# pain7576/ddpg-trucktrailer

Measured on AMD Instinct MI355X. Metric: env-steps/s, higher is better.
Workload: dtype f64

## Files before the change

ddpg-trucktrailer_amd/csrc/ttnet_pack.h:

```cpp
#pragma once
#include "ttnet_common.h"

namespace ttnet {

using f32x16 = __attribute__((ext_vector_type(16))) float;
using f16x8 = __attribute__((ext_vector_type(8))) _Float16;
using h2 = __attribute__((ext_vector_type(2))) _Float16;

constexpr int ROWS = 128, WROWS = 32;
constexpr int T1 = 13, H1P = 32 * T1;
constexpr int T2 = 10, H2P = 32 * T2;
constexpr int STEPS = H1 / 16;
constexpr int S1 = 2;
constexpr int PIECES = 2 * T2;
constexpr int CHUNK_U4 = PIECES * 64;
constexpr int CHUNK_BYTES = CHUNK_U4 * 16;
constexpr int RING = 7;
constexpr int AHEAD = RING - 2;
constexpr int RING_BYTES = RING * CHUNK_BYTES;
constexpr int W1_PIECES = S1 * T1 * 2;
constexpr int W1_BYTES = W1_PIECES * 1024;
constexpr int W1_OFF = 2 * CHUNK_BYTES;
static_assert(W1_OFF + W1_BYTES <= AHEAD * CHUNK_BYTES, "packed fc1 must fit in the ring slots that are filled after layer 1");
constexpr int VEC_FLOATS = 2 * H1P + 6 * H2P;
constexpr int VEC_PIECES = 12;
constexpr int VEC_BYTES = VEC_PIECES * 1024;
constexpr int LDS_BYTES = RING_BYTES + VEC_BYTES;
constexpr int WS_W2 = 0, WS_W1 = STEPS * CHUNK_BYTES, WS_VEC = WS_W1 + W1_BYTES, WS_BYTES = WS_VEC + VEC_BYTES;

constexpr float SX = 16.f, SW = 64.f;
constexpr float UNSCALE = 1.f / (SX * SW);

__device__ __forceinline__ void split2(const float x0, const float x1, uint32_t &ph, uint32_t &pm) {
    h2 h;
    h[0] = (_Float16)x0; h[1] = (_Float16)x1;
    ph = __builtin_bit_cast(uint32_t, h);
    float r0, r1;
    asm("v_fma_mix_f32 %0, %1, -1.0, %2 op_sel_hi:[1,0,0]" : "=v"(r0) : "v"(ph), "v"(x0));
    asm("v_fma_mix_f32 %0, %1, -1.0, %2 op_sel:[1,0,0] op_sel_hi:[1,0,0]" : "=v"(r1) : "v"(ph), "v"(x1));
    h2 m;
    m[0] = (_Float16)r0; m[1] = (_Float16)r1;
    pm = __builtin_bit_cast(uint32_t, m);
}

using f32x2 = __attribute__((ext_vector_type(2))) float;
__device__ __forceinline__ f32x2 pk(const float a, const float b) { return f32x2{a, b}; }
__device__ __forceinline__ f32x2 pk_fma(const f32x2 a, const f32x2 b, const f32x2 c) { return __builtin_elementwise_fma(a, b, c); }

__device__ __forceinline__ f32x16 mfma_f16(const uint4 a, const uint4 b, const f32x16 c) {
    return __builtin_amdgcn_mfma_f32_32x32x16_f16(__builtin_bit_cast(f16x8, a), __builtin_bit_cast(f16x8, b), c, 0, 0, 0);
}

__device__ __forceinline__ void split_pack_body(const Weights &W, const bool critic, unsigned char *__restrict__ ws,
                                                unsigned char *__restrict__ ws_alt, long long *__restrict__ bump,
                                                const RingCursor &cur, const int idx) {
    if (ws_alt && cur.k_dev && (*cur.k_dev & 1)) ws = ws_alt;
    if (idx == 0) {
        if (bump) *bump += 1;
        write_cursor(cur);
    }
    constexpr int N2 = STEPS * T2 * 64, N1 = S1 * T1 * 64;
    if (idx < N2 + N1) {
        const bool l2 = idx < N2;
        const int q = l2 ? idx : idx - N2;
        const int lane = q & 63, su = q >> 6, nt = l2 ? T2 : T1, u = su % nt, s = su / nt;
        const int r = lane & 31, h = lane >> 5, row = 32 * u + r;
        float x[8];
        if (l2) {
#pragma unroll
            for (int g = 0; g < 2; ++g) {
                const float4 v = row < H2 ? *reinterpret_cast<const float4 *>(W.w2 + (size_t)row * H1 + 16 * s + 8 * g + 4 * h)
                                          : make_float4(0.f, 0.f, 0.f, 0.f);
                x[4 * g] = v.x; x[4 * g + 1] = v.y; x[4 * g + 2] = v.z; x[4 * g + 3] = v.w;
            }
        } else {
#pragma unroll
            for (int j = 0; j < 8; ++j) {
                const int k = 16 * s + 8 * h + j;
                x[j] = row < H1 ? (k < IN ? W.w1[row * IN + k] : (k == IN ? W.b1[row] : 0.f)) : 0.f;
            }
        }
        uint32_t ph[4], pm[4];
#pragma unroll
        for (int p = 0; p < 4; ++p) split2(x[2 * p] * SW, x[2 * p + 1] * SW, ph[p], pm[p]);
        uint4 *dst = reinterpret_cast<uint4 *>(ws + (l2 ? WS_W2 : WS_W1)) + ((size_t)su * 2) * 64 + lane;
        dst[0] = make_uint4(ph[0], ph[1], ph[2], ph[3]);
        dst[64] = make_uint4(pm[0], pm[1], pm[2], pm[3]);
        return;
    }
    const int i = idx - (N2 + N1);
    if (i >= VEC_BYTES / 4) return;
    float *vec = reinterpret_cast<float *>(ws + WS_VEC);
    float v = 0.f;
    if (i < 2 * H1P) {
        const int a = i / H1P, m = i % H1P;
        if (m < H1) v = (a == 0 ? W.g1[m] : W.be1[m]) * SX;
    } else if (i < VEC_FLOATS) {
        const int a = (i - 2 * H1P) / H2P, m = (i - 2 * H1P) % H2P;
        if (m < H2) {
            const float *src[6] = {W.b2, W.g2, W.be2, W.w3, W.wa, W.ba};
            if (a < 4 || critic) v = src[a][m];
        }
    } else if (i == VEC_FLOATS) {
        v = W.b3[0];
    }
    vec[i] = v;
}
constexpr int PACK_THREADS = (STEPS * T2 + S1 * T1) * 64 + VEC_BYTES / 4;
constexpr int PACK_BLOCKS = (PACK_THREADS + 255) / 256;


}
```

ddpg-trucktrailer_amd/csrc/ttnet_split.hip:

```cpp
#include "ttnet_common.h"
#include "ttnet_pack.h"
#include "ttstamps.h"

namespace ttnet {
namespace {

#ifdef TT_STAMPS
__device__ unsigned long long g_nstamps[16];
__device__ unsigned long long g_bstamps[4096 * 8];
#define NSTAMP(i) do { if (threadIdx.x == 0) { const unsigned long long w_ = wall_clock64();                                \
        if (blockIdx.x < 4096) { g_bstamps[blockIdx.x * 8 + (i)] = w_;                                                      \
            if ((i) == 0) g_bstamps[blockIdx.x * 8 + 7] = __builtin_amdgcn_s_getreg((20 << 0) | (0 << 6) | (3 << 11)); }     \
        if (blockIdx.x == 0) { g_nstamps[i] = w_; g_nstamps[8 + i] = clock64(); } } } while (0)
__device__ unsigned long long g_tile[512][4][2];
__device__ TTLog g_log_tile;
#define TSTAMP(round, e) do { if (threadIdx.x == 0 && blockIdx.x < 512 && (round) < 4) g_tile[blockIdx.x][round][e] = wall_clock64(); } while (0)
#else
#define NSTAMP(i) do { } while (0)
#define TSTAMP(round, e) do { } while (0)
#endif

__global__ __launch_bounds__(256) void k_split_pack(const Weights W, const bool critic, unsigned char *__restrict__ ws,
                                                    unsigned char *__restrict__ ws_alt, long long *__restrict__ bump,
                                                    const RingCursor cur) {
    split_pack_body(W, critic, ws, ws_alt, bump, cur, blockIdx.x * 256 + threadIdx.x);
    publish_image(cur, PACK_BLOCKS);
}

__global__ __launch_bounds__(256) void k_pack_and_sample(const Weights W, const bool critic, unsigned char *__restrict__ ws,
                                                         unsigned char *__restrict__ ws_alt, const RingSample R,
                                                         const RingCursor cur) {
    if ((int)blockIdx.x < PACK_BLOCKS) {
        split_pack_body(W, critic, ws, ws_alt, nullptr, cur, blockIdx.x * 256 + threadIdx.x);
        publish_image(cur, PACK_BLOCKS);
        return;
    }
    const int b = ((int)blockIdx.x - PACK_BLOCKS) * 4 + (threadIdx.x >> 6);
    if (b < R.batch * R.draws) ring_sample_row(R, b, threadIdx.x & 63);
}

using lds_b = const __attribute__((address_space(3))) unsigned char;
using v4u = __attribute__((ext_vector_type(4))) unsigned;
struct LdsBases {
    lds_b *b0, *b1, *b2;
};
__device__ __forceinline__ uint4 lds_frag(const LdsBases &L, const int off) {
    lds_b *p = (off >> 16) == 0 ? L.b0 : ((off >> 16) == 1 ? L.b1 : L.b2);
    const v4u t = *(const __attribute__((address_space(3))) v4u *)(p + (off & 0xFFFF));
    return make_uint4(t[0], t[1], t[2], t[3]);
}

template <bool CRITIC>
__global__ __launch_bounds__(256, 1) void k_mlp_split(const int n, const int tile0, const int tile_end,
                                                      int *__restrict__ cursor_e, const long long *__restrict__ step_e,
                                                      const float *__restrict__ obs,
                                                      const unsigned char *__restrict__ ws,
                                                      const unsigned char *__restrict__ ws_alt,
                                                      const float *__restrict__ action, float *__restrict__ out,
                                                      const ActArgs act) {
    extern __shared__ __attribute__((aligned(16))) unsigned char lds_raw[];
    const float *p1_s = reinterpret_cast<const float *>(lds_raw + RING_BYTES);
    const int tid = threadIdx.x, lane = tid & 63;
    const int wave = __builtin_amdgcn_readfirstlane(tid >> 6);
    const int r = lane & 31, h = lane >> 5;
    using lds_f = const __attribute__((address_space(3))) float;
    using v4 = __attribute__((ext_vector_type(4))) float;
    auto lds4 = [](lds_f *q) -> float4 {
        const v4 t = *(const __attribute__((address_space(3))) v4 *)q;
        return make_float4(t[0], t[1], t[2], t[3]);
    };
    lds_f *pv1_0 = (lds_f *)(p1_s + 4 * h);
    LdsBases LB0;
    LB0.b0 = (lds_b *)lds_raw + lane * 16;
    LB0.b1 = LB0.b0 + 65536;
    LB0.b2 = LB0.b0 + 131072;
    const EpochPair epochs = await_image_early(cursor_e);
    const long long kstep = cursor_e ? *step_e : 0;
    const bool odd = act.cursor && (kstep & 1);
    const bool local = act.cursor && act.ring_slots > 0;
    const int slot_t = local ? (int)(kstep % act.ring_slots) : 0;
    const float *obs_base = local ? obs + (size_t)slot_t * act.ring_n * IN : obs;
    const unsigned lds_base0 = (unsigned)(uintptr_t)(__attribute__((address_space(3))) unsigned char *)lds_raw;
    auto dma_piece = [&](const unsigned char *base, const unsigned voff, const unsigned lds_wave, const unsigned dst_const)
                         __attribute__((always_inline)) {
        unsigned keep;
        asm volatile("s_mov_b32 %0, m0\n\ts_add_u32 m0, %3, %4\n\ts_nop 0\n\tglobal_load_lds_dwordx4 %1, %2\n\ts_mov_b32 m0, %0"
                     : "=&s"(keep) : "v"(voff), "s"(base), "s"(lds_wave), "s"(dst_const) : "memory", "scc");
    };
    const unsigned voff_w2 = lane * 16 + wave * 5120 + WS_W2;
    const unsigned voff_w1 = lane * 16 + wave * (W1_PIECES / 4) * 1024 + WS_W1;
    const unsigned voff_vec = lane * 16 + wave * (VEC_PIECES / 4) * 1024 + WS_VEC;
    const unsigned ldsw_w2_0 = lds_base0 + wave * 5120, ldsw_w1_0 = lds_base0 + W1_OFF + wave * (W1_PIECES / 4) * 1024;
    auto issue_fc1 = [&](const unsigned char *w, const unsigned ldsw_w1) __attribute__((always_inline)) {
#pragma unroll
        for (int i = 0; i < W1_PIECES / 4; ++i) dma_piece(w, voff_w1 + i * 1024, ldsw_w1, i * 1024);
    };
    auto issue_step_piece = [&](const unsigned char *w, const unsigned ldsw_w2, const int s, const int i) __attribute__((always_inline)) {
        dma_piece(w, voff_w2 + s * CHUNK_BYTES + i * 1024, ldsw_w2, (s % RING) * CHUNK_BYTES + i * 1024);
    };
    float xo[S1][8];
    float ou_pre = 0.f;
    unsigned dp_pre = 0u;
    const bool with_noise = !CRITIC && act.ou != nullptr;
    const uint8_t *dprev = act.done_prev;
    float *araw = act.act_raw;
    auto load_obs = [&](const int tile) __attribute__((always_inline)) {
        const int row = tile * ROWS + wave * WROWS + r;
        const int rowc = row < n ? row : n - 1;
        const float *orow = obs_base + (size_t)rowc * IN;
#pragma unroll
        for (int s = 0; s < S1; ++s)
#pragma unroll
            for (int j = 0; j < 8; ++j) {
                const int k = 16 * s + 8 * h + j;
                xo[s][j] = orow[k < IN ? k : IN - 1];
            }
        if (with_noise) {
            ou_pre = act.ou[rowc];
            dp_pre = dprev ? (unsigned)dprev[rowc] : 0u;
        }
    };

    NSTAMP(0);
    int tile = tile0 + (int)blockIdx.x;
    if (tile >= tile_end) return;
    if (local) {
        const int sl = act.ring_slots;
        const int slot_prev = slot_t == 0 ? sl - 1 : slot_t - 1;
        dprev = kstep > 0 ? act.done_prev + (size_t)slot_prev * act.ring_n : nullptr;
        araw = act.act_raw + (size_t)slot_t * act.ring_n;
    }
    if (!act.cursor || local) load_obs(tile);
    await_image(act.cursor, act.step_dev, epochs);
    const unsigned char *wsl = (odd && ws_alt) ? ws_alt : ws;
    if (act.cursor && !local) {
        obs_base = resolve_obs(act, obs);
        const int *c = cursor_of(act);
        dprev = c[3] ? act.done_prev + (size_t)c[2] * act.ring_n : nullptr;
        araw = act.act_raw + (size_t)c[0] * act.ring_n;
        load_obs(tile);
    }
    const unsigned long long noise_step = act.step + (act.step_dev ? (unsigned long long)*act.step_dev : 0ull);
    if (act.cursor && tile0 == 0 && blockIdx.x == 0 && tid == 0)
        __hip_atomic_store(act.cursor + CUR_PROGRESS, (int)(kstep + 1), __ATOMIC_RELAXED, __HIP_MEMORY_SCOPE_AGENT);
    if (act.cursor && tile0 == 0 && blockIdx.x == 0 && tid < 4) {
        const int sl = act.ring_slots;
        act.cursor[tid] = !local ? cursor_of(act)[tid]
                                 : (tid == 0 ? slot_t : tid == 1 ? (slot_t + 1 == sl ? 0 : slot_t + 1)
                                                      : tid == 2 ? (slot_t == 0 ? sl - 1 : slot_t - 1) : (kstep > 0 ? 1 : 0));
    }
    issue_fc1(wsl, ldsw_w1_0);
#pragma unroll
    for (int i = 0; i < VEC_PIECES / 4; ++i)
        dma_piece(wsl, voff_vec + i * 1024, lds_base0 + RING_BYTES + wave * (VEC_PIECES / 4) * 1024, i * 1024);
#pragma unroll
    for (int i = 0; i < 10; ++i) issue_step_piece(wsl, ldsw_w2_0, i / 5, i % 5);
    bool first = true;
#ifdef TT_STAMPS
    int round = 0;
    if (threadIdx.x == 0 && blockIdx.x < 512) for (int q = 0; q < 4; ++q) g_tile[blockIdx.x][q][0] = g_tile[blockIdx.x][q][1] = 0ull;
    if (threadIdx.x == 0 && blockIdx.x < 512) g_tile[blockIdx.x][0][0] = wall_clock64();
#endif

#pragma unroll 1
    for (;;) {
        const unsigned char *wsl_cur = wsl;
        unsigned ldsw_w2 = ldsw_w2_0, ldsw_w1 = ldsw_w1_0;
        LdsBases LB = LB0;
        lds_f *pv1 = pv1_0;
        asm volatile("" : "+s"(wsl_cur), "+s"(ldsw_w2), "+s"(ldsw_w1), "+v"(LB.b0), "+v"(LB.b1), "+v"(LB.b2), "+v"(pv1));
        lds_f *pv2 = pv1 + 2 * H1P;
        const int row = tile * ROWS + wave * WROWS + r;
#pragma unroll
        for (int s = 0; s < S1; ++s)
#pragma unroll
            for (int j = 0; j < 8; ++j) {
                const int k = 16 * s + 8 * h + j;
                xo[s][j] = k < IN ? (row < n ? xo[s][j] : 0.f) : (k == IN ? 1.f : 0.f);
            }
        float ou_next = 0.f;
        if (with_noise) ou_next = ou_advance(row < n ? row : n - 1, ou_pre, dp_pre != 0u, act, noise_step);
        uint4 xb[S1][2];
#pragma unroll
        for (int s = 0; s < S1; ++s) {
            uint32_t ph[4], pm[4];
#pragma unroll
            for (int p = 0; p < 4; ++p) split2(xo[s][2 * p] * SX, xo[s][2 * p + 1] * SX, ph[p], pm[p]);
            xb[s][0] = make_uint4(ph[0], ph[1], ph[2], ph[3]);
            xb[s][1] = make_uint4(pm[0], pm[1], pm[2], pm[3]);
        }
        if (first) asm volatile("s_waitcnt vmcnt(10)" ::: "memory");
        else asm volatile("s_waitcnt vmcnt(0)" ::: "memory");
        __builtin_amdgcn_s_barrier();
        if (first) NSTAMP(1);

        f32x16 acc1[T1];
#pragma unroll
        for (int t = 0; t < T1; ++t) {
#pragma unroll
            for (int v = 0; v < 16; ++v) acc1[t][v] = 0.f;
#pragma unroll
            for (int s = 0; s < S1; ++s) {
                const uint4 ah = lds_frag(LB, W1_OFF + ((s * T1 + t) * 2) * 1024), am = lds_frag(LB, W1_OFF + ((s * T1 + t) * 2 + 1) * 1024);
                acc1[t] = mfma_f16(am, xb[s][0], acc1[t]);
                acc1[t] = mfma_f16(ah, xb[s][1], acc1[t]);
                acc1[t] = mfma_f16(ah, xb[s][0], acc1[t]);
            }
        }
        if (first) NSTAMP(2);
        __builtin_amdgcn_s_barrier();
#pragma unroll
        for (int i = 10; i < 5 * (AHEAD + 1); ++i) issue_step_piece(wsl_cur, ldsw_w2, i / 5, i % 5);
        uint32_t hb[STEPS][4], mb[STEPS][4];
        f32x2 nmean, rstdp;
        {
            f32x2 sp = pk(0.f, 0.f);
#pragma unroll
            for (int t = 0; t < T1; ++t)
#pragma unroll
                for (int v = 0; v < (t == T1 - 1 ? 8 : 16); v += 4)
                    sp += pk(acc1[t][v], acc1[t][v + 1]) + pk(acc1[t][v + 2], acc1[t][v + 3]);
            const float s = sp[0] + sp[1];
            const float mean = (s + __shfl_xor(s, 32)) * (1.f / H1);
            nmean = pk(-mean, -mean);
            f32x2 ssp = pk(0.f, 0.f);
#pragma unroll
            for (int t = 0; t < T1; ++t)
#pragma unroll
                for (int v = 0; v < (t == T1 - 1 ? 8 : 16); v += 2) {
                    const f32x2 d = pk(acc1[t][v], acc1[t][v + 1]) + nmean;
                    ssp = pk_fma(d, d, ssp);
                }
            const float ss = ssp[0] + ssp[1];
            const float var = (ss + __shfl_xor(ss, 32)) * (1.f / H1) * (UNSCALE * UNSCALE);
            const float rstd = rsqrtf(var + 1e-5f) * UNSCALE;
            rstdp = pk(rstd, rstd);
        }
        constexpr int GROUPS = 2 * STEPS;
        float4 gq[2], bq[2];
        f32x2 ya, yb;
        float y0, y1, y2, y3;
        auto ln_read = [&](const int G) __attribute__((always_inline)) {
            gq[G & 1] = lds4(pv1 + 8 * G);
            bq[G & 1] = lds4(pv1 + H1P + 8 * G);
        };
        auto ln_chunk = [&](const int G, const int k) __attribute__((always_inline)) {
            const int t = G >> 2, i = G & 3, st = G >> 1, e = 2 * (G & 1);
            const float4 g = gq[G & 1], be = bq[G & 1];
            if (k == 0) ya = pk_fma((pk(acc1[t][4 * i], acc1[t][4 * i + 1]) + nmean) * rstdp, pk(g.x, g.y), pk(be.x, be.y));
            if (k == 1) yb = pk_fma((pk(acc1[t][4 * i + 2], acc1[t][4 * i + 3]) + nmean) * rstdp, pk(g.z, g.w), pk(be.z, be.w));
            if (k == 2) {
                y0 = fmaxf(ya[0], 0.f); y1 = fmaxf(ya[1], 0.f); y2 = fmaxf(yb[0], 0.f); y3 = fmaxf(yb[1], 0.f);
                if (G + 1 < GROUPS) ln_read(G + 1);
            }
            if (k == 3) split2(y0, y1, hb[st][e], mb[st][e]);
            if (k == 4) split2(y2, y3, hb[st][e + 1], mb[st][e + 1]);
        };
        ln_read(0);
#pragma unroll
        for (int G = 0; G < 4; ++G)
#pragma unroll
            for (int k = 0; k < 5; ++k) ln_chunk(G, k);

        if (first) NSTAMP(3);
        f32x16 acc2[T2];
#pragma unroll
        for (int u = 0; u < T2; ++u)
#pragma unroll
            for (int v = 0; v < 16; ++v) acc2[u][v] = 0.f;
#define SB __builtin_amdgcn_sched_barrier(0)
        asm volatile("s_waitcnt vmcnt(20)" ::: "memory");
        __builtin_amdgcn_s_barrier();
        uint4 c0h = lds_frag(LB, 0), c0m = lds_frag(LB, 1024), c1h = lds_frag(LB, 2048), c1m = lds_frag(LB, 3072), c2h = c0h, c2m = c0m;
        SB;
#pragma unroll
        for (int s = 0; s < STEPS; ++s) {
            const uint4 vh = make_uint4(hb[s][0], hb[s][1], hb[s][2], hb[s][3]), vm = make_uint4(mb[s][0], mb[s][1], mb[s][2], mb[s][3]);
            const int slot = (s % RING) * CHUNK_BYTES, nslot = ((s + 1) % RING) * CHUNK_BYTES;
            const unsigned char *wsl_s = wsl_cur;
            unsigned lds_s = ldsw_w2;
            asm volatile("" : "+s"(wsl_s), "+s"(lds_s));
#pragma unroll
            for (int u = 0; u < T2; ++u) {
                if (u == T2 / 2) {
                    switch (STEPS - 2 - s < 4 ? STEPS - 2 - s : 4) {
                        case 4: asm volatile("s_waitcnt vmcnt(20)" ::: "memory"); break;
                        case 3: asm volatile("s_waitcnt vmcnt(15)" ::: "memory"); break;
                        case 2: asm volatile("s_waitcnt vmcnt(10)" ::: "memory"); break;
                        case 1: asm volatile("s_waitcnt vmcnt(5)" ::: "memory"); break;
                        default: asm volatile("s_waitcnt vmcnt(0)" ::: "memory"); break;
                    }
                    __builtin_amdgcn_s_barrier();
                    SB;
                }
                const bool more = u + 2 < T2 || s + 1 < STEPS;
                const int nx = u + 2 < T2 ? slot + (u + 2) * 2048 : nslot + (u + 2 - T2) * 2048;
                acc2[u] = mfma_f16(c0h, vm, acc2[u]); SB;
                if (more) c2h = lds_frag(LB, nx);
                if (s + 2 < STEPS) ln_chunk(2 * (s + 2) + u / 5, u % 5);
                SB;
                acc2[u] = mfma_f16(c0m, vh, acc2[u]); SB;
                if (more) c2m = lds_frag(LB, nx + 1024);
                SB;
                acc2[u] = mfma_f16(c0h, vh, acc2[u]); SB;
                if (u >= 5 && s + RING - 1 < STEPS) issue_step_piece(wsl_s, lds_s, s + RING - 1, u - 5);
                SB;
                c0h = c1h; c0m = c1m; c1h = c2h; c1m = c2m;
            }
        }
#undef SB

        if (first) NSTAMP(4);
        const int next = tile + (int)gridDim.x;
        const bool more_tiles = next < tile_end;
        if (more_tiles) {
            __builtin_amdgcn_s_barrier();
            load_obs(next);
            issue_fc1(wsl_cur, ldsw_w1);
#pragma unroll
            for (int i = 0; i < 10; ++i) issue_step_piece(wsl_cur, ldsw_w2, i / 5, i % 5);
        }
        f32x2 s2p = pk(0.f, 0.f);
        {
            float4 bq[2][4];
            auto ldb = [&](const int u, float4 (&b)[4]) {
#pragma unroll
                for (int i = 0; i < 4; ++i) b[i] = lds4(pv2 + 32 * u + 8 * i);
            };
            ldb(0, bq[0]);
#pragma unroll
            for (int u = 0; u < T2; ++u) {
                if (u + 1 < T2) ldb(u + 1, bq[(u + 1) & 1]);
                __builtin_amdgcn_sched_barrier(0);
#pragma unroll
                for (int i = 0; i < 4; ++i) {
                    const float4 b = bq[u & 1][i];
                    const f32x2 xa = pk_fma(pk(acc2[u][4 * i], acc2[u][4 * i + 1]), pk(UNSCALE, UNSCALE), pk(b.x, b.y));
                    const f32x2 xb2 = pk_fma(pk(acc2[u][4 * i + 2], acc2[u][4 * i + 3]), pk(UNSCALE, UNSCALE), pk(b.z, b.w));
                    acc2[u][4 * i] = xa[0]; acc2[u][4 * i + 1] = xa[1]; acc2[u][4 * i + 2] = xb2[0]; acc2[u][4 * i + 3] = xb2[1];
                    s2p += xa + xb2;
                }
                __builtin_amdgcn_sched_barrier(0);
            }
        }
        const float s2 = s2p[0] + s2p[1];
        const float mean2 = (s2 + __shfl_xor(s2, 32)) * (1.f / H2);
        const f32x2 nmean2 = pk(-mean2, -mean2);
        f32x2 ss2p = pk(0.f, 0.f);
#pragma unroll
        for (int u = 0; u < T2; ++u)
#pragma unroll
            for (int i = 0; i < 4; ++i) {
                const bool real = 32 * u + 8 * i + 4 * h < H2;
                const f32x2 keep = real ? pk(1.f, 1.f) : pk(0.f, 0.f);
#pragma unroll
                for (int j = 0; j < 4; j += 2) {
                    const f32x2 d = pk(acc2[u][4 * i + j], acc2[u][4 * i + j + 1]) + nmean2;
                    acc2[u][4 * i + j] = d[0]; acc2[u][4 * i + j + 1] = d[1];
                    const f32x2 dk = (32 * u + 8 * i + 4 < H2) ? d : d * keep;
                    ss2p = pk_fma(dk, dk, ss2p);
                }
            }
        const float ss2 = ss2p[0] + ss2p[1];
        const float rstd2 = rsqrtf((ss2 + __shfl_xor(ss2, 32)) * (1.f / H2) + 1e-5f);
        const f32x2 rstd2p = pk(rstd2, rstd2);
        const float av = (CRITIC && row < n) ? action[row] : 0.f;
        f32x2 dotp = pk(0.f, 0.f);
        {
            constexpr int NV = CRITIC ? 5 : 3;
            float4 vq[2][4][NV];
            auto ldv = [&](const int u, float4 (&v)[4][NV]) {
#pragma unroll
                for (int i = 0; i < 4; ++i)
#pragma unroll
                    for (int q = 0; q < NV; ++q) v[i][q] = lds4(pv2 + (q + 1) * H2P + 32 * u + 8 * i);
            };
            ldv(0, vq[0]);
#pragma unroll
            for (int u = 0; u < T2; ++u) {
                if (u + 1 < T2) ldv(u + 1, vq[(u + 1) & 1]);
                __builtin_amdgcn_sched_barrier(0);
#pragma unroll
                for (int i = 0; i < 4; ++i) {
                    const float4 g = vq[u & 1][i][0], be = vq[u & 1][i][1], w3 = vq[u & 1][i][2];
                    f32x2 ya = pk_fma(pk(acc2[u][4 * i], acc2[u][4 * i + 1]) * rstd2p, pk(g.x, g.y), pk(be.x, be.y));
                    f32x2 yb = pk_fma(pk(acc2[u][4 * i + 2], acc2[u][4 * i + 3]) * rstd2p, pk(g.z, g.w), pk(be.z, be.w));
                    if (CRITIC) {
                        const float4 wa = vq[u & 1][i][NV - 2], ba = vq[u & 1][i][NV - 1];
                        ya += pk_fma(pk(av, av), pk(wa.x, wa.y), pk(ba.x, ba.y));
                        yb += pk_fma(pk(av, av), pk(wa.z, wa.w), pk(ba.z, ba.w));
                    }
                    dotp = pk_fma(pk(fmaxf(ya[0], 0.f), fmaxf(ya[1], 0.f)), pk(w3.x, w3.y), dotp);
                    dotp = pk_fma(pk(fmaxf(yb[0], 0.f), fmaxf(yb[1], 0.f)), pk(w3.z, w3.w), dotp);
                }
                __builtin_amdgcn_sched_barrier(0);
            }
        }
        const float dot = dotp[0] + dotp[1];
        const float v = dot + __shfl_xor(dot, 32) + lds4(pv1 - 4 * h + VEC_FLOATS).x;
        if (h == 0 && row < n) {
            if (with_noise) finish_row_noise(row, v, out, act, ou_next, araw);
            else finish_row<CRITIC>(row, v, out, act);
        }
        if (first) NSTAMP(5);
#ifdef TT_STAMPS
        TSTAMP(round, 1);
        if (threadIdx.x == 0 && blockIdx.x < 512 && round < 4) tt_log_add(g_log_tile, g_tile[blockIdx.x][round][0], g_tile[blockIdx.x][round][1]);
        ++round;
        if (more_tiles) TSTAMP(round, 0);
#endif
        if (!more_tiles) break;
        tile = next;
        first = false;
    }
}

}

#ifdef TT_STAMPS
int split_debug_stamps(unsigned long long *out16) {
    return hipMemcpyFromSymbol(out16, HIP_SYMBOL(g_nstamps), sizeof(unsigned long long) * 16) == hipSuccess ? 0 : -3;
}
int split_debug_tiles(unsigned long long *out4096) {
    return hipMemcpyFromSymbol(out4096, HIP_SYMBOL(g_tile), sizeof(unsigned long long) * 512 * 4 * 2) == hipSuccess ? 0 : -3;
}
int split_debug_log(unsigned long long *out, int reset) {
    if (out && hipMemcpyFromSymbol(out, HIP_SYMBOL(g_log_tile), sizeof(TTLog)) != hipSuccess) return -3;
    if (reset) { const unsigned long long z = 0; if (hipMemcpyToSymbol(HIP_SYMBOL(g_log_tile), &z, sizeof(z)) != hipSuccess) return -3; }
    return 0;
}
int split_debug_poll(unsigned long long *out4) {
    return hipMemcpyFromSymbol(out4, HIP_SYMBOL(g_poll), sizeof(unsigned long long) * 4) == hipSuccess ? 0 : -3;
}
int split_debug_block_stamps(unsigned long long *out, int nblocks) {
    return hipMemcpyFromSymbol(out, HIP_SYMBOL(g_bstamps), sizeof(unsigned long long) * 8 * (nblocks < 4096 ? nblocks : 4096)) == hipSuccess ? 0 : -3;
}
#endif

size_t split_ws_bytes() { return (size_t)WS_BYTES; }

int split_pack(const tt_mlp_weights *w, bool critic, void *ws, long long *bump, const RingCursor &cur, hipStream_t stream) {
    unsigned char *alt = ws == w->split_ws ? reinterpret_cast<unsigned char *>(w->split_ws_alt) : nullptr;
    hipLaunchKernelGGL(k_split_pack, dim3(PACK_BLOCKS), dim3(256), 0, stream, to_weights(w), critic,
                       reinterpret_cast<unsigned char *>(ws), alt, bump, cur);
    return hipGetLastError() == hipSuccess ? TT_OK : TT_EHIP;
}

int split_pack_and_sample(const tt_mlp_weights *w, bool critic, void *ws, const RingSample &R, const RingCursor &cur,
                          hipStream_t stream) {
    unsigned char *alt = ws == w->split_ws ? reinterpret_cast<unsigned char *>(w->split_ws_alt) : nullptr;
    hipLaunchKernelGGL(k_pack_and_sample, dim3(PACK_BLOCKS + (R.batch * R.draws + 3) / 4), dim3(256), 0, stream, to_weights(w), critic,
                       reinterpret_cast<unsigned char *>(ws), alt, R, cur);
    return hipGetLastError() == hipSuccess ? TT_OK : TT_EHIP;
}

template <bool CRITIC>
static int launch_split(int n, const float *obs, const float *action, const tt_mlp_weights *w, float *out,
                        const ActArgs &act, hipStream_t stream) {
    static bool attr[64] = {};
    static int cus[64] = {};
    int dev = 0;
    if (hipGetDevice(&dev) != hipSuccess || dev < 0 || dev >= 64) return TT_EHIP;
    if (!attr[dev]) {
        if (hipFuncSetAttribute(reinterpret_cast<const void *>(&k_mlp_split<CRITIC>),
                                hipFuncAttributeMaxDynamicSharedMemorySize, LDS_BYTES) != hipSuccess)
            return TT_EHIP;
        int c = 0;
        if (hipDeviceGetAttribute(&c, hipDeviceAttributeMultiprocessorCount, dev) != hipSuccess || c <= 0) c = 256;
        cus[dev] = c;
        attr[dev] = true;
    }
    const int ntiles = (n + ROWS - 1) / ROWS;
    const int chip = cus[dev];
    int capped = 0;
    if (w->max_workgroups > 0) {
        const int limit = w->max_workgroups;
        capped = ntiles;
        if (w->capped_grids > 0 && (long long)w->capped_grids * limit < ntiles) capped = w->capped_grids * limit;
        const int rounds = (capped + limit - 1) / limit, g = (capped + rounds - 1) / rounds;
        hipLaunchKernelGGL((k_mlp_split<CRITIC>), dim3(g), dim3(256), LDS_BYTES, stream, n, 0, capped, act.cursor, act.step_dev, obs,
                           reinterpret_cast<const unsigned char *>(w->split_ws),
                           reinterpret_cast<const unsigned char *>(w->split_ws_alt), action, out, act);
    }
    if (capped < ntiles) {
        const int rest = ntiles - capped, rounds = (rest + chip - 1) / chip, g = (rest + rounds - 1) / rounds;
        hipLaunchKernelGGL((k_mlp_split<CRITIC>), dim3(g), dim3(256), LDS_BYTES, stream, n, capped, ntiles, act.cursor, act.step_dev, obs,
                           reinterpret_cast<const unsigned char *>(w->split_ws),
                           reinterpret_cast<const unsigned char *>(w->split_ws_alt), action, out, act);
    }
    return hipGetLastError() == hipSuccess ? TT_OK : TT_EHIP;
}

int split_forward(bool critic, int n, const float *obs, const float *action, const tt_mlp_weights *w, float *out,
                  const ActArgs &act, hipStream_t stream) {
    return critic ? launch_split<true>(n, obs, action, w, out, act, stream)
                  : launch_split<false>(n, obs, action, w, out, act, stream);
}

}
```

Baseline: 793.1 million.

## Interleave weight DMA issue into fc1 and fc2 MFMA loops with static schedule

Moves the packed fc1 weights to ring slots 4..6 and spreads their async global-to-LDS loads, plus the first layer-2 chunks and the next tile's prefetch, across the MFMA loops using a compile-time job table. Layer 1 gets a software-pipelined fragment loop that issues weight pieces between MFMAs, and the barrier-plus-burst issue between layers and tiles is removed. The counted vmcnt waits are derived from the schedule and checked with static_asserts. A 32-bit modulo fast path is also added for the slot index. This adds scheduling complexity and risks LDS overwrite hazards if the slot analysis is wrong.

New measurement: 826.8 million (median of 6 runs). 4.3% higher.

```diff
diff --git a/ddpg-trucktrailer_amd/csrc/ttnet_pack.h b/ddpg-trucktrailer_amd/csrc/ttnet_pack.h
--- a/ddpg-trucktrailer_amd/csrc/ttnet_pack.h
+++ b/ddpg-trucktrailer_amd/csrc/ttnet_pack.h
@@ -20,8 +20,10 @@
 constexpr int RING_BYTES = RING * CHUNK_BYTES;
 constexpr int W1_PIECES = S1 * T1 * 2;
 constexpr int W1_BYTES = W1_PIECES * 1024;
-constexpr int W1_OFF = 2 * CHUNK_BYTES;
-static_assert(W1_OFF + W1_BYTES <= AHEAD * CHUNK_BYTES, "packed fc1 must fit in the ring slots that are filled after layer 1");
+constexpr int W1_OFF = 4 * CHUNK_BYTES;
+constexpr int W1_WAVE_PIECES = W1_PIECES / 4;
+static_assert(W1_OFF + W1_BYTES <= RING_BYTES, "packed fc1 must fit in ring slots 4..6");
+static_assert(W1_OFF % CHUNK_BYTES == 0 && CHUNK_BYTES % 4096 == 0, "a slot holds whole rows of four pieces (one per wave)");
 constexpr int VEC_FLOATS = 2 * H1P + 6 * H2P;
 constexpr int VEC_PIECES = 12;
 constexpr int VEC_BYTES = VEC_PIECES * 1024;
diff --git a/ddpg-trucktrailer_amd/csrc/ttnet_split.hip b/ddpg-trucktrailer_amd/csrc/ttnet_split.hip
--- a/ddpg-trucktrailer_amd/csrc/ttnet_split.hip
+++ b/ddpg-trucktrailer_amd/csrc/ttnet_split.hip
@@ -38,6 +38,59 @@
     const int b = ((int)blockIdx.x - PACK_BLOCKS) * 4 + (threadIdx.x >> 6);
     if (b < R.batch * R.draws) ring_sample_row(R, b, threadIdx.x & 63);
 }
+
+constexpr int JOB_NONE = -1, JOB_FC1 = 100, JOB_NEXT = 200;
+constexpr int TAIL0 = STEPS - (RING - 1);
+constexpr int l2_job(const int s, const int u) {
+    if (s == 0) return AHEAD - 1 + u / 5;
+    if (s == 1 && u < 5) return RING - 1;
+    if (u < 5) return JOB_NONE;
+    if (s < TAIL0) return s + RING - 1;
+    const int i = 5 * (s - TAIL0) + u - 5;
+    if (i < W1_WAVE_PIECES) return JOB_FC1 + i;
+    if (s == TAIL0 + 3 || s == TAIL0 + 4) return JOB_NEXT + s - (TAIL0 + 3);
+    return JOB_NONE;
+}
+constexpr int l2_piece(const int u) { return u % 5; }
+constexpr int job_slot(const int j) { return j >= JOB_NEXT ? j - JOB_NEXT : (j >= JOB_FC1 ? W1_OFF / CHUNK_BYTES + (j - JOB_FC1) / 5 : j % RING); }
+constexpr bool l2_slots_free() {
+    for (int s = 0; s < STEPS; ++s)
+        for (int u = 0; u < T2; ++u) {
+            const int j = l2_job(s, u);
+            if (j == JOB_NONE) continue;
+            if (s == 0 || (s == 1 && u < 5)) { if (job_slot(j) < W1_OFF / CHUNK_BYTES) return false; }
+            else if (u < 5 || job_slot(j) != (s - 1) % RING) return false;
+        }
+    return true;
+}
+static_assert(l2_slots_free(), "a piece of layer 2 overwrites a slot that may still be read");
+constexpr int mid_allowed(const int s) {
+    int n = 10, after = s + 1 == 2 ? 5 : (s + 1 == 3 ? 10 : -1000);
+    for (int ss = 0; ss < STEPS; ++ss)
+        for (int u = 0; u < T2; ++u) {
+            if (ss == s && u == T2 / 2) return n - after;
+            const int j = l2_job(ss, u);
+            if (j != JOB_NONE) { ++n; if (j == s + 1) after = n; }
+        }
+    return -1;
+}
+constexpr bool mid_counts_ok() {
+    for (int s = 1; s + 1 < STEPS; ++s) if (mid_allowed(s) != (s < TAIL0 + 3 ? 20 : 18)) return false;
+    return true;
+}
+static_assert(mid_counts_ok(), "the counted waits of layer 2 do not match the issue schedule");
+struct L2Schedule {
+    int job[STEPS][T2], mid[STEPS];
+};
+constexpr L2Schedule make_l2_schedule() {
+    L2Schedule t{};
+    for (int s = 0; s < STEPS; ++s) {
+        t.mid[s] = mid_allowed(s);
+        for (int u = 0; u < T2; ++u) t.job[s][u] = l2_job(s, u);
+    }
+    return t;
+}
+constexpr L2Schedule L2S = make_l2_schedule();
 
 using lds_b = const __attribute__((address_space(3))) unsigned char;
 using v4u = __attribute__((ext_vector_type(4))) unsigned;
@@ -78,7 +131,8 @@
     const long long kstep = cursor_e ? *step_e : 0;
     const bool odd = act.cursor && (kstep & 1);
     const bool local = act.cursor && act.ring_slots > 0;
-    const int slot_t = local ? (int)(kstep % act.ring_slots) : 0;
+    const int slot_t = !local ? 0 : ((unsigned long long)kstep >> 32) == 0ull ? (int)((unsigned)kstep % (unsigned)act.ring_slots)
+                                                                             : (int)(kstep % act.ring_slots);
     const float *obs_base = local ? obs + (size_t)slot_t * act.ring_n * IN : obs;
     const unsigned lds_base0 = (unsigned)(uintptr_t)(__attribute__((address_space(3))) unsigned char *)lds_raw;
     auto dma_piece = [&](const unsigned char *base, const unsigned voff, const unsigned lds_wave, const unsigned dst_const)
@@ -88,12 +142,11 @@
                      : "=&s"(keep) : "v"(voff), "s"(base), "s"(lds_wave), "s"(dst_const) : "memory", "scc");
     };
     const unsigned voff_w2 = lane * 16 + wave * 5120 + WS_W2;
-    const unsigned voff_w1 = lane * 16 + wave * (W1_PIECES / 4) * 1024 + WS_W1;
+    const unsigned voff_w1 = lane * 16 + wave * 1024 + WS_W1;
     const unsigned voff_vec = lane * 16 + wave * (VEC_PIECES / 4) * 1024 + WS_VEC;
-    const unsigned ldsw_w2_0 = lds_base0 + wave * 5120, ldsw_w1_0 = lds_base0 + W1_OFF + wave * (W1_PIECES / 4) * 1024;
-    auto issue_fc1 = [&](const unsigned char *w, const unsigned ldsw_w1) __attribute__((always_inline)) {
-#pragma unroll
-        for (int i = 0; i < W1_PIECES / 4; ++i) dma_piece(w, voff_w1 + i * 1024, ldsw_w1, i * 1024);
+    const unsigned ldsw_w2_0 = lds_base0 + wave * 5120, ldsw_w1_0 = lds_base0 + W1_OFF + wave * 1024;
+    auto issue_fc1_piece = [&](const unsigned char *w, const unsigned ldsw_w1, const int i) __attribute__((always_inline)) {
+        dma_piece(w, voff_w1 + i * 4096, ldsw_w1, i * 4096);
     };
     auto issue_step_piece = [&](const unsigned char *w, const unsigned ldsw_w2, const int s, const int i) __attribute__((always_inline)) {
         dma_piece(w, voff_w2 + s * CHUNK_BYTES + i * 1024, ldsw_w2, (s % RING) * CHUNK_BYTES + i * 1024);
@@ -149,12 +202,11 @@
                                  : (tid == 0 ? slot_t : tid == 1 ? (slot_t + 1 == sl ? 0 : slot_t + 1)
                                                       : tid == 2 ? (slot_t == 0 ? sl - 1 : slot_t - 1) : (kstep > 0 ? 1 : 0));
     }
-    issue_fc1(wsl, ldsw_w1_0);
+#pragma unroll
+    for (int i = 0; i < W1_WAVE_PIECES; ++i) issue_fc1_piece(wsl, ldsw_w1_0, i);
 #pragma unroll
     for (int i = 0; i < VEC_PIECES / 4; ++i)
         dma_piece(wsl, voff_vec + i * 1024, lds_base0 + RING_BYTES + wave * (VEC_PIECES / 4) * 1024, i * 1024);
-#pragma unroll
-    for (int i = 0; i < 10; ++i) issue_step_piece(wsl, ldsw_w2_0, i / 5, i % 5);
     bool first = true;
 #ifdef TT_STAMPS
     int round = 0;
@@ -189,28 +241,41 @@
             xb[s][0] = make_uint4(ph[0], ph[1], ph[2], ph[3]);
             xb[s][1] = make_uint4(pm[0], pm[1], pm[2], pm[3]);
         }
-        if (first) asm volatile("s_waitcnt vmcnt(10)" ::: "memory");
-        else asm volatile("s_waitcnt vmcnt(0)" ::: "memory");
+        asm volatile("s_waitcnt vmcnt(0)" ::: "memory");
         __builtin_amdgcn_s_barrier();
         if (first) NSTAMP(1);
 
+#define SB __builtin_amdgcn_sched_barrier(0)
         f32x16 acc1[T1];
-#pragma unroll
-        for (int t = 0; t < T1; ++t) {
-#pragma unroll
-            for (int v = 0; v < 16; ++v) acc1[t][v] = 0.f;
-#pragma unroll
-            for (int s = 0; s < S1; ++s) {
-                const uint4 ah = lds_frag(LB, W1_OFF + ((s * T1 + t) * 2) * 1024), am = lds_frag(LB, W1_OFF + ((s * T1 + t) * 2 + 1) * 1024);
-                acc1[t] = mfma_f16(am, xb[s][0], acc1[t]);
-                acc1[t] = mfma_f16(ah, xb[s][1], acc1[t]);
-                acc1[t] = mfma_f16(ah, xb[s][0], acc1[t]);
+        {
+            auto w1_frag = [&](const int q, const int plane) __attribute__((always_inline)) {
+                return lds_frag(LB, W1_OFF + (((q % S1) * T1 + q / S1) * 2 + plane) * 1024);
+            };
+            const unsigned char *wsl_1 = wsl_cur;
+            asm volatile("" : "+s"(wsl_1));
+            uint4 a0h = w1_frag(0, 0), a0m = w1_frag(0, 1), a1h = w1_frag(1, 0), a1m = w1_frag(1, 1), a2h = a0h, a2m = a0m;
+            SB;
+#pragma unroll
+            for (int q = 0; q < S1 * T1; ++q) {
+                const int t = q / S1, s = q % S1;
+                if (s == 0) {
+#pragma unroll
+                    for (int v = 0; v < 16; ++v) acc1[t][v] = 0.f;
+                }
+                acc1[t] = mfma_f16(a0m, xb[s][0], acc1[t]); SB;
+                if (q + 2 < S1 * T1) a2h = w1_frag(q + 2, 0);
+                SB;
+                acc1[t] = mfma_f16(a0h, xb[s][1], acc1[t]); SB;
+                if (q + 2 < S1 * T1) a2m = w1_frag(q + 2, 1);
+                SB;
+                acc1[t] = mfma_f16(a0h, xb[s][0], acc1[t]); SB;
+                if (q < 10) { if (first) issue_step_piece(wsl_1, ldsw_w2, q / 5, q % 5); }
+                else if (q < 20) issue_step_piece(wsl_1, ldsw_w2, 2 + (q - 10) / 5, q % 5);
+                SB;
+                a0h = a1h; a0m = a1m; a1h = a2h; a1m = a2m;
             }
         }
         if (first) NSTAMP(2);
-        __builtin_amdgcn_s_barrier();
-#pragma unroll
-        for (int i = 10; i < 5 * (AHEAD + 1); ++i) issue_step_piece(wsl_cur, ldsw_w2, i / 5, i % 5);
         uint32_t hb[STEPS][4], mb[STEPS][4];
         f32x2 nmean, rstdp;
         {
@@ -268,27 +333,23 @@
         for (int u = 0; u < T2; ++u)
 #pragma unroll
             for (int v = 0; v < 16; ++v) acc2[u][v] = 0.f;
-#define SB __builtin_amdgcn_sched_barrier(0)
-        asm volatile("s_waitcnt vmcnt(20)" ::: "memory");
+        asm volatile("s_waitcnt vmcnt(10)" ::: "memory");
         __builtin_amdgcn_s_barrier();
         uint4 c0h = lds_frag(LB, 0), c0m = lds_frag(LB, 1024), c1h = lds_frag(LB, 2048), c1m = lds_frag(LB, 3072), c2h = c0h, c2m = c0m;
         SB;
-#pragma unroll
-        for (int s = 0; s < STEPS; ++s) {
+        auto l2_step = [&](const int s) __attribute__((always_inline)) {
             const uint4 vh = make_uint4(hb[s][0], hb[s][1], hb[s][2], hb[s][3]), vm = make_uint4(mb[s][0], mb[s][1], mb[s][2], mb[s][3]);
             const int slot = (s % RING) * CHUNK_BYTES, nslot = ((s + 1) % RING) * CHUNK_BYTES;
             const unsigned char *wsl_s = wsl_cur;
-            unsigned lds_s = ldsw_w2;
+            unsigned lds_s = ldsw_w2, lds1_s = ldsw_w1;
             asm volatile("" : "+s"(wsl_s), "+s"(lds_s));
+            if (s >= TAIL0 && s < TAIL0 + 3) asm volatile("" : "+s"(lds1_s));
 #pragma unroll
             for (int u = 0; u < T2; ++u) {
-                if (u == T2 / 2) {
-                    switch (STEPS - 2 - s < 4 ? STEPS - 2 - s : 4) {
-                        case 4: asm volatile("s_waitcnt vmcnt(20)" ::: "memory"); break;
-                        case 3: asm volatile("s_waitcnt vmcnt(15)" ::: "memory"); break;
-                        case 2: asm volatile("s_waitcnt vmcnt(10)" ::: "memory"); break;
-                        case 1: asm volatile("s_waitcnt vmcnt(5)" ::: "memory"); break;
-                        default: asm volatile("s_waitcnt vmcnt(0)" ::: "memory"); break;
+                if (u == T2 / 2 && s >= 1 && s + 1 < STEPS) {
+                    switch (L2S.mid[s]) {
+                        case 20: asm volatile("s_waitcnt vmcnt(20)" ::: "memory"); break;
+                        default: asm volatile("s_waitcnt vmcnt(18)" ::: "memory"); break;
                     }
                     __builtin_amdgcn_s_barrier();
                     SB;
@@ -303,23 +364,30 @@
                 if (more) c2m = lds_frag(LB, nx + 1024);
                 SB;
                 acc2[u] = mfma_f16(c0h, vh, acc2[u]); SB;
-                if (u >= 5 && s + RING - 1 < STEPS) issue_step_piece(wsl_s, lds_s, s + RING - 1, u - 5);
+                {
+                    const int j = L2S.job[s][u];
+                    const bool f1 = j >= JOB_FC1 && j < JOB_NEXT;
+                    const int st = j >= JOB_NEXT ? j - JOB_NEXT : j, i1 = j - JOB_FC1;
+                    if (j != JOB_NONE)
+                        dma_piece(wsl_s, f1 ? voff_w1 + i1 * 4096 : voff_w2 + st * CHUNK_BYTES + l2_piece(u) * 1024, f1 ? lds1_s : lds_s,
+                                  f1 ? i1 * 4096 : (st % RING) * CHUNK_BYTES + l2_piece(u) * 1024);
+                }
                 SB;
                 c0h = c1h; c0m = c1m; c1h = c2h; c1m = c2m;
             }
-        }
+        };
+#pragma unroll
+        for (int s = 0; s < 2; ++s) l2_step(s);
+#pragma unroll
+        for (int s = 2; s < TAIL0; ++s) l2_step(s);
+#pragma unroll
+        for (int s = TAIL0; s < STEPS; ++s) l2_step(s);
 #undef SB
 
         if (first) NSTAMP(4);
         const int next = tile + (int)gridDim.x;
         const bool more_tiles = next < tile_end;
-        if (more_tiles) {
-            __builtin_amdgcn_s_barrier();
-            load_obs(next);
-            issue_fc1(wsl_cur, ldsw_w1);
-#pragma unroll
-            for (int i = 0; i < 10; ++i) issue_step_piece(wsl_cur, ldsw_w2, i / 5, i % 5);
-        }
+        if (more_tiles) load_obs(next);
         f32x2 s2p = pk(0.f, 0.f);
         {
             float4 bq[2][4];
@@ -413,6 +481,7 @@
         tile = next;
         first = false;
     }
+    asm volatile("s_waitcnt vmcnt(0)" ::: "memory");
 }
 
 }
```
